# graphdeco-inria/hierarchical-3d-gaussians

Measured on NVIDIA H100. Metric: train-step images/sec (fwd+bwd) @1080p, 3M Gaussians, SH-3, higher is better.
Workload: dtype f32

## Files before the change

hierarchical-3d-gaussians_b200/csrc/common.cuh:

```cuda
#pragma once
#include <cuda_runtime.h>
#include <stdint.h>
#include <stdio.h>
#include <stdlib.h>
#include "../../include/h3dgs.h"

namespace h3dgs {

constexpr float kNearPlane = 0.2f;
constexpr float kFovClamp = 1.3f;
constexpr float kDilation = 0.3f;
constexpr float kLambdaFloor = 0.1f;
constexpr int kTile = H3DGS_TILE;
constexpr int kTilePixels = kTile * kTile;
constexpr float kAlphaCap = 0.99f;
constexpr float kAlphaSkip = 1.0f / 255.0f;
constexpr float kTStop = 0.0001f;
constexpr float kWEps = 0.0000001f;
constexpr uint32_t kKidsMask = 0xFFFFFu;
constexpr int kClampShift = 20;
constexpr uint32_t kSortedKidsMask = 0xFFFu;
constexpr int kBlockShift = 16;

struct __align__(16) Record { float4 a, b, c; };
static_assert(sizeof(Record) == 48, "record must be 48 bytes");

__host__ __device__ inline size_t align_up(size_t x, size_t a = 256) { return (x + a - 1) / a * a; }

struct GeomLayout {
    size_t depths, tiles_touched, offsets, rank_mask, records, scan_temp, total;
    size_t scan_temp_bytes;
};
struct BinLayout {
    size_t keys_unsorted, keys_sorted, vals_unsorted, vals_sorted, sort_temp, sorted_records, total;
    size_t sort_temp_bytes;
};
struct ImgLayout {
    size_t final_T, n_contrib, ranges, tile_max_contrib, tile_count, scan_info, total;
};
struct ScanInfo { uint32_t D, max_count, overflow, prefilter_bad; };
constexpr int kTileSortCap = 8192;

GeomLayout geom_layout(int P);
BinLayout bin_layout(int64_t D);
ImgLayout img_layout(int W, int H);

void prof_begin(int stage, cudaStream_t s);
void prof_end(int stage, cudaStream_t s);
struct ProfScope {
    int stage; cudaStream_t s;
    ProfScope(int st, cudaStream_t ss) : stage(st), s(ss) { prof_begin(stage, s); }
    ~ProfScope() { prof_end(stage, s); }
};

int pinned_scratch(void** out);

void set_error(const char* fmt, ...);
extern int64_t g_launches;

#define H3_CUDA(call)                                                                      \
    do {                                                                                   \
        cudaError_t e__ = (call);                                                          \
        if (e__ != cudaSuccess) {                                                          \
            h3dgs::set_error("%s failed at %s:%d: %s", #call, __FILE__, __LINE__,          \
                             cudaGetErrorString(e__));                                     \
            return H3DGS_ECUDA;                                                            \
        }                                                                                  \
    } while (0)

#define H3_LAUNCHED(name, debug, stream)                                                   \
    do {                                                                                   \
        h3dgs::g_launches++;                                                               \
        cudaError_t e__ = cudaGetLastError();                                              \
        if (e__ == cudaSuccess && (debug)) e__ = cudaStreamSynchronize(stream);            \
        if (e__ != cudaSuccess) {                                                          \
            h3dgs::set_error("kernel %s failed: %s", name, cudaGetErrorString(e__));       \
            return H3DGS_ECUDA;                                                            \
        }                                                                                  \
    } while (0)

int launch_preprocess(const h3dgs_raster_args& a, int32_t* radii, float* depths, uint32_t* tiles_touched,
                      uint8_t* rank_mask, Record* records, uint32_t* tile_count, ScanInfo* info, cudaStream_t s);
int launch_tile_scan(const h3dgs_raster_args& a, const uint32_t* tile_count, uint32_t* ranges, ScanInfo* info,
                     uint32_t cap_entries, uint32_t cap_list, cudaStream_t s);
int launch_tile_binning(const h3dgs_raster_args& a, const int32_t* radii, const float* depths, const Record* records,
                        int64_t D, uint32_t max_count, uint8_t* bin, const BinLayout& bl, const uint32_t* ranges,
                        const ScanInfo* info, uint32_t* tile_count, cudaStream_t s);
int launch_preprocess_color(const h3dgs_raster_args& a, const int32_t* radii, const uint32_t* tiles_touched,
                            Record* records, cudaStream_t s);
int launch_sh_backward(const h3dgs_raster_args& a, const int32_t* radii, const uint8_t* rank_mask, const Record* records,
                       const float* accum, float* dL_dmeans3D, float* dL_dsh, cudaStream_t s);
int launch_scan(const uint32_t* in, uint32_t* out, int n, void* temp, size_t temp_bytes, cudaStream_t s, bool debug);
size_t scan_temp_bytes(int n);
size_t sort_temp_bytes(int64_t n);
int launch_binning(const h3dgs_raster_args& a, const int32_t* radii, const float* depths, const uint32_t* offsets,
                   const Record* records, int64_t D, uint8_t* bin, const BinLayout& bl, uint32_t* ranges,
                   cudaStream_t s);
int launch_render_forward(const h3dgs_raster_args& a, const uint32_t* ranges, const Record* sorted_records,
                          float* out_color, float* out_invdepth, float* final_T, uint32_t* n_contrib,
                          uint32_t* tile_max_contrib, cudaStream_t s);
int launch_render_backward(const h3dgs_raster_args& a, const uint32_t* ranges, const Record* sorted_records,
                           const uint32_t* point_list, const float* final_T, const uint32_t* n_contrib,
                           const uint32_t* tile_max_contrib, const float* dL_dcolor, const float* dL_dinvdepth,
                           float* accum , cudaStream_t s);
int launch_preprocess_backward(const h3dgs_raster_args& a, const int32_t* radii, const uint8_t* rank_mask, const Record* records,
                               const float* accum, float* dL_dmeans3D, float* dL_dmeans2D, float* dL_dsh,
                               float* dL_dcolors, float* dL_dopacities, float* dL_dscales, float* dL_drots,
                               float* dL_dcov3D, cudaStream_t s);

#ifdef __CUDACC__
__device__ __forceinline__ void quad_pixel(int tile_x, int tile_y, int warp, int lane, int& px, int& py0) {
    px = tile_x * kTile + 8 * (warp & 1) + (lane & 7);
    py0 = tile_y * kTile + 8 * (warp >> 1) + 2 * (lane >> 3);
}

__device__ __forceinline__ void group_pixel(int tile_x, int tile_y, int warp, int lane, int& px, int& py0) {
    const int g = lane >> 3, k = lane & 7;
    px = tile_x * kTile + 8 * (warp & 1) + 4 * (g & 1) + (k & 3);
    py0 = tile_y * kTile + 8 * (warp >> 1) + 4 * (g >> 1) + 2 * (k >> 2);
}
inline bool use_group_walk() { const char* e = getenv("H3DGS_GROUPWALK"); return !(e && e[0] == '0'); }

#endif

struct PeerPtrs { void* p[H3DGS_MAX_PEERS]; int n; };
inline PeerPtrs peer_ptrs(void* const* src, int n) {
    PeerPtrs r; r.n = n > 1 ? n : 0;
    for (int k = 0; k < H3DGS_MAX_PEERS; k++) r.p[k] = (k < r.n) ? src[k] : nullptr;
    return r;
}
struct RowCycle { int shift, world, rank; };
inline RowCycle row_cycle(const h3dgs_raster_args& a) {
    RowCycle c; c.world = a.peer_count > 1 ? a.peer_count : 0; c.rank = a.shard_index; c.shift = a.grad_cyclic_log2;
    return c;
}
inline int cyclic_local_rows(const RowCycle& c, int P) {
    const int blocks = (P + (1 << c.shift) - 1) >> c.shift;
    return ((blocks + c.world - 1 - c.rank) / c.world) << c.shift;
}
#ifdef __CUDACC__
__device__ __forceinline__ int cyclic_row(const RowCycle& c, int local) {
    return ((((local >> c.shift) * c.world + c.rank)) << c.shift) + (local & ((1 << c.shift) - 1));
}
__device__ __forceinline__ bool cyclic_owned(const RowCycle& c, int row) { return ((row >> c.shift) % c.world) == c.rank; }
#endif

#ifdef __CUDACC__
struct StagePtrs { const float* own; const float* stage; int n, rank; size_t slot_floats; };
template <int NPAIR>
__device__ __forceinline__ void gather_accum_pairs(const StagePtrs& sp, uint32_t mask, int i, int first, float (&out)[2 * NPAIR]) {
#pragma unroll
    for (int k = 0; k < 2 * NPAIR; k++) out[k] = 0.f;
#pragma unroll
    for (int r = 0; r < H3DGS_MAX_PEERS; r++) {
        if (r < sp.n && ((mask >> r) & 1u)) {
            const float* row = (r == sp.rank ? sp.own : sp.stage + (size_t)r * sp.slot_floats) + (size_t)i * 10 + 2 * first;
#pragma unroll
            for (int k = 0; k < NPAIR; k++) {
                const float2 v = __ldcg(reinterpret_cast<const float2*>(row + 2 * k));
                out[2 * k] += v.x; out[2 * k + 1] += v.y;
            }
        }
    }
}
#endif
inline StagePtrs stage_ptrs(const h3dgs_raster_args& a, const float* accum) {
    StagePtrs sp; sp.own = accum; sp.n = a.peer_count > 1 ? a.peer_count : 0; sp.rank = a.shard_index;
    sp.stage = sp.n ? static_cast<const float*>(a.peer_stage[a.shard_index]) : nullptr;
    sp.slot_floats = (size_t)a.P * 10;
    return sp;
}
int launch_peer_push(const h3dgs_raster_args& a, const uint8_t* rank_mask, const float* accum, cudaStream_t s);

#ifdef H3_SIMT_EMU
extern long long g_emu_stats[16];
#define H3_STAT(i, n) (h3dgs::g_emu_stats[i] += (n))
#else
#define H3_STAT(i, n) ((void)0)
#endif

constexpr int kAccum = 10;

}

#ifdef __CUDACC__
#include "pair_math.cuh"
#endif
```

hierarchical-3d-gaussians_b200/csrc/pair_math.cuh:

```cuda
#pragma once

#ifdef H3_PAIR_HOST_EMU
#include <math.h>
#include <stdint.h>
#define H3_PM_FN static inline
namespace h3dgs {
#ifndef H3_SIMT_EMU
struct float4 { float x, y, z, w; };
constexpr float kAlphaCap = 0.99f;
constexpr float kAlphaSkip = 1.0f / 255.0f;
constexpr float kTStop = 0.0001f;
constexpr uint32_t kSortedKidsMask = 0xFFFu;
#endif
struct f2 { float lo, hi; };
H3_PM_FN f2 pk(float lo, float hi) { return f2{lo, hi}; }
H3_PM_FN void upk(f2 v, float& lo, float& hi) { lo = v.lo; hi = v.hi; }
H3_PM_FN f2 fma2(f2 a, f2 b, f2 c) { return f2{fmaf(a.lo, b.lo, c.lo), fmaf(a.hi, b.hi, c.hi)}; }
H3_PM_FN f2 mul2(f2 a, f2 b) { return f2{a.lo * b.lo, a.hi * b.hi}; }
H3_PM_FN f2 add2(f2 a, f2 b) { return f2{a.lo + b.lo, a.hi + b.hi}; }
H3_PM_FN f2 sub2(f2 a, f2 b) { return f2{a.lo - b.lo, a.hi - b.hi}; }
H3_PM_FN float fast_exp2(float x) { return exp2f(x); }
H3_PM_FN float fast_log2(float x) { return log2f(x); }
H3_PM_FN float rcp_approx(float x) { return 1.0f / x; }
H3_PM_FN float rsq_approx(float x) { return 1.0f / sqrtf(x); }
#else
#define H3_PM_FN __device__ __forceinline__
namespace h3dgs {
struct f2 { float lo, hi; };
H3_PM_FN f2 pk(float lo, float hi) { return f2{lo, hi}; }
H3_PM_FN void upk(f2 v, float& lo, float& hi) { lo = v.lo; hi = v.hi; }
H3_PM_FN f2 fma2(f2 a, f2 b, f2 c) { return f2{__fmaf_rn(a.lo, b.lo, c.lo), __fmaf_rn(a.hi, b.hi, c.hi)}; }
H3_PM_FN f2 mul2(f2 a, f2 b) { return f2{__fmul_rn(a.lo, b.lo), __fmul_rn(a.hi, b.hi)}; }
H3_PM_FN f2 add2(f2 a, f2 b) { return f2{__fadd_rn(a.lo, b.lo), __fadd_rn(a.hi, b.hi)}; }
H3_PM_FN f2 sub2(f2 a, f2 b) { return f2{__fsub_rn(a.lo, b.lo), __fsub_rn(a.hi, b.hi)}; }
H3_PM_FN float fast_exp2(float x) { float y; asm("ex2.approx.ftz.f32 %0, %1;" : "=f"(y) : "f"(x)); return y; }
H3_PM_FN float fast_log2(float x) { float y; asm("lg2.approx.ftz.f32 %0, %1;" : "=f"(y) : "f"(x)); return y; }
H3_PM_FN float rcp_approx(float x) { float y; asm("rcp.approx.ftz.f32 %0, %1;" : "=f"(y) : "f"(x)); return y; }
H3_PM_FN float rsq_approx(float x) { float y; asm("rsqrt.approx.ftz.f32 %0, %1;" : "=f"(y) : "f"(x)); return y; }
#endif

H3_PM_FN f2 bc(float x) { return pk(x, x); }
H3_PM_FN float lo(f2 v) { float a, b; upk(v, a, b); return a; }
H3_PM_FN float hi(f2 v) { float a, b; upk(v, a, b); return b; }
H3_PM_FN float hsum(f2 v) { float a, b; upk(v, a, b); return a + b; }
H3_PM_FN f2 sel2(bool p0, bool p1, f2 x, f2 y) {
    float x0, x1, y0, y1; upk(x, x0, x1); upk(y, y0, y1);
    return pk(p0 ? x0 : y0, p1 ? x1 : y1);
}
H3_PM_FN f2 ex2_2(f2 v) { float a, b; upk(v, a, b); return pk(fast_exp2(a), fast_exp2(b)); }
H3_PM_FN float fast_rcp(float x) { const float r = rcp_approx(x); return r * (2.0f - x * r); }
H3_PM_FN f2 rcp2(f2 x) {
    float x0, x1; upk(x, x0, x1);
    const f2 r = pk(rcp_approx(x0), rcp_approx(x1));
    return mul2(r, sub2(bc(2.0f), mul2(x, r)));
}

H3_PM_FN f2 pair_power(const float4& a, const float4& bb, float dx, f2 nfpy, f2& d) {
    d = add2(bc(a.y), nfpy);
    const float A = (a.z * dx) * (dx * -0.5f), B = -a.w * dx, C = -0.5f * bb.x;
    return fma2(fma2(bc(C), d, bc(B)), d, bc(A));
}
H3_PM_FN void pair_gauss(f2 power, float opacity, f2& G, f2& abase) {
    G = ex2_2(mul2(power, bc(1.4426950408889634f)));
    float a0, a1; upk(mul2(bc(opacity), G), a0, a1);
    abase = pk(fminf(kAlphaCap, a0), fminf(kAlphaCap, a1));
}
template <bool HIER, bool GRAD>
H3_PM_FN void pair_hier_alpha(f2 a, float t, uint32_t k , f2& alpha, f2& dadb) {
    alpha = a; dadb = bc(1.0f);
    if (!HIER) return;
    if (k <= 1u || t >= 1.0f) return;
    const float u = 1.0f - t;
    float a0, a1; upk(a, a0, a1);
    float o0, o1; upk(sub2(bc(1.0f), a), o0, o1);
    if (k == 2u) {
        const f2 r = pk(rsq_approx(o0), rsq_approx(o1));
        const f2 s = mul2(pk(o0, o1), r);
        f2 S = fma2(a, bc(0.02734375f), bc(0.0390625f));
        S = fma2(a, S, bc(0.0625f));
        S = fma2(a, S, bc(0.125f));
        S = fma2(a, S, bc(0.5f));
        const f2 omr = sel2(a0 < 0.0625f, a1 < 0.0625f, mul2(a, S), sub2(bc(1.0f), s));
        alpha = fma2(bc(u), omr, mul2(bc(t), a));
        if (GRAD) dadb = fma2(bc(0.5f * u), r, bc(t));
        return;
    }
    const float ik = fast_rcp((float)k);
    const f2 l2 = pk(fast_log2(o0), fast_log2(o1));
    f2 L = fma2(a, bc(0.2f), bc(0.25f));
    L = fma2(a, L, bc(0.33333334f));
    L = fma2(a, L, bc(0.5f));
    L = fma2(a, L, bc(1.0f));
    const f2 yn = mul2(mul2(a, L), bc(ik));
    f2 S = fma2(yn, bc(-0.041666668f), bc(0.16666667f));
    S = fma2(yn, S, bc(-0.5f));
    S = fma2(yn, S, bc(1.0f));
    const f2 omr_series = mul2(yn, S);
    const f2 omr_mufu = sub2(bc(1.0f), ex2_2(mul2(l2, bc(ik))));
    const f2 omr = sel2(a0 < 0.0625f, a1 < 0.0625f, omr_series, omr_mufu);
    alpha = fma2(bc(u), omr, mul2(bc(t), a));
    if (GRAD) dadb = fma2(bc(u * ik), ex2_2(mul2(l2, bc(ik - 1.0f))), bc(t));
}

H3_PM_FN f2 pair_blend(f2 pw, f2 al, f2& T, bool& done0, bool& done1, bool& v0, bool& v1, bool active = true) {
    const f2 tT = mul2(T, sub2(bc(1.0f), al));
    float pw0, pw1, al0, al1, tT0, tT1;
    upk(pw, pw0, pw1); upk(al, al0, al1); upk(tT, tT0, tT1);
    v0 = active && !done0 && pw0 <= 0.0f && al0 >= kAlphaSkip;
    v1 = active && !done1 && pw1 <= 0.0f && al1 >= kAlphaSkip;
    if (v0 && tT0 < kTStop) { done0 = true; v0 = false; }
    if (v1 && tT1 < kTStop) { done1 = true; v1 = false; }
    const f2 w = sel2(v0, v1, mul2(al, T), bc(0.f));
    T = sel2(v0, v1, tT, T);
    return w;
}

struct PairState { f2 T, acc; };

template <bool HIER, bool DEPTH>
H3_PM_FN void pair_grad(const float4& a, const float4& bb, float dx, f2 d, f2 G, f2 alpha, f2 dadb, f2 cg, f2 T_final,
                        f2 neg_bg_dot, f2 g0, f2 g1, f2 g2, f2 gd, PairState& st, float (&v)[10])
{
    const f2 rcp = rcp2(sub2(bc(1.0f), alpha));
    const f2 Tn = mul2(st.T, rcp);
    const f2 diff = sub2(cg, st.acc);
    const f2 dL_dalpha = fma2(mul2(T_final, rcp), neg_bg_dot, mul2(diff, Tn));
    const f2 dL_dab = HIER ? mul2(dL_dalpha, dadb) : dL_dalpha;
    const f2 w = mul2(alpha, Tn);
    st.T = Tn;
    st.acc = fma2(alpha, diff, st.acc);
    const f2 dL_dG = mul2(bc(bb.y), dL_dab);
    const f2 gdx = mul2(G, bc(dx)), gdy = mul2(G, d);
    const f2 qx = mul2(gdx, dL_dG), qy = mul2(gdy, dL_dG);
    v[0] = hsum(fma2(qy, bc(-a.w), mul2(qx, bc(-a.z))));
    v[1] = hsum(fma2(qx, bc(-a.w), mul2(qy, bc(-bb.x))));
    v[2] = hsum(qx) * dx;
    v[3] = hsum(mul2(qx, d));
    v[4] = hsum(mul2(qy, d));
    v[5] = hsum(mul2(G, dL_dab));
    v[6] = hsum(mul2(w, g0)); v[7] = hsum(mul2(w, g1)); v[8] = hsum(mul2(w, g2));
    v[9] = DEPTH ? hsum(mul2(w, gd)) : 0.f;
}

}
#undef H3_PM_FN
```

hierarchical-3d-gaussians_b200/csrc/render_backward.cu:

```cuda
#include "common.cuh"
#include "tma.cuh"

namespace h3dgs {

#ifdef H3_BLEND_OCC8
constexpr int kBwdBatch = 224;
constexpr int kBwdMinBlocks = 8;
#else
constexpr int kBwdBatch = 256;
constexpr int kBwdMinBlocks = 1;
#endif
constexpr int kBwdStages = 2;

__device__ __forceinline__ int reduce_slot(int lane) {
    if (lane & 1) return -1;
    const int b4 = (lane >> 4) & 1, b3 = (lane >> 3) & 1, b2 = (lane >> 2) & 1, b1 = (lane >> 1) & 1;
    int ai;
    if (!b3) { if (b2 && b1) return -1; ai = b2 ? 2 : b1; }
    else     { if (b2) return -1; ai = 3 + b1; }
    return 5 * b4 + ai;
}
__device__ __forceinline__ float xchg_add(float keep, float send, int mask) {
    return keep + __shfl_xor_sync(0xffffffffu, send, mask);
}
__device__ __forceinline__ f2 xchg_add2(float keep0, float send0, float keep1, float send1, int mask) {
    return add2(pk(keep0, keep1), pk(__shfl_xor_sync(0xffffffffu, send0, mask), __shfl_xor_sync(0xffffffffu, send1, mask)));
}
__device__ __forceinline__ float transpose_reduce10(const float (&v)[10], int lane) {
    const bool b4 = lane & 16, b3 = lane & 8, b2 = lane & 4, b1 = lane & 2;
    float a[5];
    upk(xchg_add2(b4 ? v[5] : v[0], b4 ? v[0] : v[5], b4 ? v[6] : v[1], b4 ? v[1] : v[6], 16), a[0], a[1]);
    upk(xchg_add2(b4 ? v[7] : v[2], b4 ? v[2] : v[7], b4 ? v[8] : v[3], b4 ? v[3] : v[8], 16), a[2], a[3]);
    a[4] = xchg_add(b4 ? v[9] : v[4], b4 ? v[4] : v[9], 16);
    float b[3];
    upk(xchg_add2(b3 ? a[3] : a[0], b3 ? a[0] : a[3], b3 ? a[4] : a[1], b3 ? a[1] : a[4], 8), b[0], b[1]);
    b[2] = xchg_add(b3 ? 0.f : a[2], b3 ? a[2] : 0.f, 8);
    float c[2];
    upk(xchg_add2(b2 ? b[2] : b[0], b2 ? b[0] : b[2], b2 ? 0.f : b[1], b2 ? b[1] : 0.f, 4), c[0], c[1]);
    float d = xchg_add(b1 ? c[1] : c[0], b1 ? c[0] : c[1], 2);
    d += __shfl_xor_sync(0xffffffffu, d, 1);
    return d;
}

__device__ __forceinline__ void group_slots(int k, int& s0, int& s1) {
    const int b2 = (k >> 2) & 1, b1 = (k >> 1) & 1, b0 = k & 1, base = 5 * b2;
    if (!b0) { s0 = base + (b1 ? 3 : 0); s1 = base + (b1 ? 4 : 1); }
    else { s0 = b1 ? -1 : base + 2; s1 = -1; }
}
__device__ __forceinline__ void transpose_reduce10_g8(const float (&v)[10], int lane, float& r0, float& r1) {
    const bool b2 = lane & 4, b1 = lane & 2, b0 = lane & 1;
    float a[5];
    upk(xchg_add2(b2 ? v[5] : v[0], b2 ? v[0] : v[5], b2 ? v[6] : v[1], b2 ? v[1] : v[6], 4), a[0], a[1]);
    upk(xchg_add2(b2 ? v[7] : v[2], b2 ? v[2] : v[7], b2 ? v[8] : v[3], b2 ? v[3] : v[8], 4), a[2], a[3]);
    a[4] = xchg_add(b2 ? v[9] : v[4], b2 ? v[4] : v[9], 4);
    float b[3];
    upk(xchg_add2(b1 ? a[3] : a[0], b1 ? a[0] : a[3], b1 ? a[4] : a[1], b1 ? a[1] : a[4], 2), b[0], b[1]);
    b[2] = xchg_add(b1 ? 0.f : a[2], b1 ? a[2] : 0.f, 2);
    upk(xchg_add2(b0 ? b[2] : b[0], b0 ? b[0] : b[2], b0 ? 0.f : b[1], b0 ? b[1] : 0.f, 1), r0, r1);
}

constexpr int kBwdThreads = 128;

template <bool HIER, bool DEPTH, bool GROUPS>
__global__ void __launch_bounds__(kBwdThreads, kBwdMinBlocks)
render_backward_kernel(int W, int H, int gx, int shard_count, int shard_index, const uint2* __restrict__ ranges,
                       const Record* __restrict__ sorted, const uint32_t* __restrict__ point_list,
                       const float* __restrict__ bg, const float* __restrict__ final_T,
                       const uint32_t* __restrict__ n_contrib, const uint32_t* __restrict__ tile_max_contrib,
                       const float* __restrict__ dL_dcolor, const float* __restrict__ dL_dinvdepth,
                       float* __restrict__ accum)
{
    __shared__ __align__(128) Record s_rec[kBwdStages][kBwdBatch];
    __shared__ uint32_t s_id[kBwdStages][kBwdBatch];
    __shared__ __align__(8) uint64_t s_full[kBwdStages];
    __shared__ uint8_t s_list[GROUPS ? kBwdThreads / 32 : 1][4][GROUPS ? kBwdBatch : 4];

    const int tid = threadIdx.x, lane = tid & 31, warp = tid >> 5;
    const int slot = reduce_slot(lane);
    const int tile_x = blockIdx.x % gx;
    const int tile_y = (blockIdx.x / gx) * shard_count + shard_index;
    const int tile = tile_y * gx + tile_x;
    const uint2 range = ranges[tile];
    const int n = min((int)(range.y - range.x), (int)tile_max_contrib[tile]);
    const int nb = (n + kBwdBatch - 1) / kBwdBatch;
    if (nb == 0) return;
    const Record* src = sorted + range.x;
    const uint32_t* ids = point_list + range.x;

    auto stage_ids = [&](int it) {
        const int b = nb - 1 - it, st = it % kBwdStages;
        for (int k = tid; k < kBwdBatch; k += kBwdThreads) {
            const int e = b * kBwdBatch + k;
            if (e < n) s_id[st][k] = ids[e];
        }
    };
    for (int it = 0; it < kBwdStages && it < nb; it++) stage_ids(it);
    if (tid == 0) {
        for (int s = 0; s < kBwdStages; s++) mbar_init(&s_full[s], 1);
        fence_mbar_init();
    }
    __syncthreads();
    auto issue = [&](int it) {
        const int b = nb - 1 - it, st = it % kBwdStages;
        const uint32_t bytes = (uint32_t)min(kBwdBatch, n - b * kBwdBatch) * (uint32_t)sizeof(Record);
        mbar_arrive_expect_tx(&s_full[st], bytes);
        tma_load_1d(&s_rec[st][0], src + (size_t)b * kBwdBatch, bytes, &s_full[st]);
    };
    if (tid == 0)
        for (int it = 0; it < kBwdStages && it < nb; it++) issue(it);

    int px, py0;
    if (GROUPS) group_pixel(tile_x, tile_y, warp, lane, px, py0);
    else quad_pixel(tile_x, tile_y, warp, lane, px, py0);
    int gs0, gs1;
    group_slots(lane & 7, gs0, gs1);
    const int grp = lane >> 3;
    const int py1 = py0 + 1;
    const bool in0 = px < W && py0 < H, in1 = px < W && py1 < H;
    const float fpx = (float)px;
    const f2 nfpy = pk(-(float)py0, -(float)py1);
    const size_t pix0 = (size_t)py0 * W + px, pix1 = (size_t)py1 * W + px, plane = (size_t)H * W;
    const float Tf0 = in0 ? final_T[pix0] : 0.f, Tf1 = in1 ? final_T[pix1] : 0.f;
    const f2 Tf = pk(Tf0, Tf1);
    PairState ps = {Tf, bc(0.f)};
    const int last0 = in0 ? (int)n_contrib[pix0] : 0, last1 = in1 ? (int)n_contrib[pix1] : 0;
    float ga0 = 0.f, ga1 = 0.f, ga2 = 0.f, gad = 0.f, gb0 = 0.f, gb1 = 0.f, gb2 = 0.f, gbd = 0.f;
    if (in0) { ga0 = dL_dcolor[pix0]; ga1 = dL_dcolor[plane + pix0]; ga2 = dL_dcolor[2 * plane + pix0]; if (DEPTH) gad = dL_dinvdepth[pix0]; }
    if (in1) { gb0 = dL_dcolor[pix1]; gb1 = dL_dcolor[plane + pix1]; gb2 = dL_dcolor[2 * plane + pix1]; if (DEPTH) gbd = dL_dinvdepth[pix1]; }
    const f2 g0 = pk(ga0, gb0), g1 = pk(ga1, gb1), g2 = pk(ga2, gb2), gd = pk(gad, gbd);
    const f2 neg_bgd = pk(-(bg[0] * ga0 + bg[1] * ga1 + bg[2] * ga2), -(bg[0] * gb0 + bg[1] * gb1 + bg[2] * gb2));
    const int wlast = (int)__reduce_max_sync(0xffffffffu, (unsigned)max(last0, last1));
    const int qsel = kBlockShift + 4 * warp;
    int gl0, gl1, gl2, gl3;
    {
        int gm = max(last0, last1);
        gm = max(gm, __shfl_xor_sync(0xffffffffu, gm, 4)); gm = max(gm, __shfl_xor_sync(0xffffffffu, gm, 2));
        gm = max(gm, __shfl_xor_sync(0xffffffffu, gm, 1));
        gl0 = __shfl_sync(0xffffffffu, gm, 0); gl1 = __shfl_sync(0xffffffffu, gm, 8);
        gl2 = __shfl_sync(0xffffffffu, gm, 16); gl3 = __shfl_sync(0xffffffffu, gm, 24);
    }

    for (int it = 0; it < nb; it++) {
        const int st = it % kBwdStages, b = nb - 1 - it;
        mbar_wait(&s_full[st], (uint32_t)((it / kBwdStages) & 1));
        const int cnt = min(kBwdBatch, n - b * kBwdBatch);
        const Record* rec = &s_rec[st][0];
        auto replay_entry = [&](int j, bool has) {
            const int e = b * kBwdBatch + j;
            const float4 a = rec[j].a;
            const float4 bb = rec[j].b;
            const uint32_t gid = s_id[st][j];
            const uint32_t kb = __float_as_uint(bb.w);
            const float dx = a.x - fpx;
            f2 d, G, al, dadb = bc(1.0f);
            const f2 pw = pair_power(a, bb, dx, nfpy, d);
            pair_gauss(pw, bb.y, G, al);
            float pw0, pw1, al0, al1;
            upk(pw, pw0, pw1); upk(al, al0, al1);
            bool v0 = has && e < last0 && pw0 <= 0.0f && al0 >= kAlphaSkip;
            bool v1 = has && e < last1 && pw1 <= 0.0f && al1 >= kAlphaSkip;
            if (lane == 0) H3_STAT(0, 1);
            if ((lane & 7) == 0 && has) H3_STAT(3, 1);
            if (!__any_sync(0xffffffffu, v0 || v1)) { if (lane == 0) H3_STAT(1, 1); return; }
            if (HIER) {
                pair_hier_alpha<HIER, true>(al, bb.z, kb & kSortedKidsMask, al, dadb);
                upk(al, al0, al1);
                v0 = v0 && al0 >= kAlphaSkip;
                v1 = v1 && al1 >= kAlphaSkip;
            }
            H3_STAT(2, (v0 ? 1 : 0) + (v1 ? 1 : 0));
#ifdef H3_SIMT_EMU
            { const uint32_t tk = __ballot_sync(0xffffffffu, v0 || v1);
              if (GROUPS && (lane & 7) == 0 && has && ((tk >> (8 * grp)) & 0xFFu) == 0u) H3_STAT(4, 1); }
#endif
            G = sel2(v0, v1, G, bc(0.f));
            al = sel2(v0, v1, al, bc(0.f));
            const float4 c = rec[j].c;
            f2 cg = fma2(bc(c.z), g2, fma2(bc(c.y), g1, mul2(bc(c.x), g0)));
            if (DEPTH) cg = fma2(bc(c.w), gd, cg);
            float v[10];
            pair_grad<HIER, DEPTH>(a, bb, dx, d, G, al, dadb, cg, Tf, neg_bgd, g0, g1, g2, gd, ps, v);
            if (GROUPS) {
                const bool taker = ((__ballot_sync(0xffffffffu, v0 || v1) >> (8 * grp)) & 0xFFu) != 0u;
                float r0, r1;
                transpose_reduce10_g8(v, lane, r0, r1);
                float* row = accum + (size_t)gid * kAccum;
                if (taker && gs0 >= 0 && (DEPTH || gs0 < 9)) atomicAdd(row + gs0, r0);
                if (taker && gs1 >= 0 && (DEPTH || gs1 < 9)) atomicAdd(row + gs1, r1);
            } else {
                const float total = transpose_reduce10(v, lane);
                float* row = accum + (size_t)gid * kAccum;
                if (slot >= 0 && (DEPTH || slot < 9)) atomicAdd(row + slot, total);
            }
        };
        if (GROUPS) {
            uint8_t* lst = &s_list[warp][0][0];
            const uint32_t lt = (1u << lane) - 1u;
            int c0 = 0, c1 = 0, c2 = 0, c3 = 0;
            for (int j0 = 0; j0 < cnt; j0 += 32) {
                const int jl = j0 + lane, e = b * kBwdBatch + jl;
                uint32_t nib = jl < cnt ? (__float_as_uint(rec[jl].b.w) >> qsel) & 0xFu : 0u;
                nib &= (e < gl0 ? 1u : 0u) | (e < gl1 ? 2u : 0u) | (e < gl2 ? 4u : 0u) | (e < gl3 ? 8u : 0u);
                const uint32_t m0 = __ballot_sync(0xffffffffu, nib & 1u), m1 = __ballot_sync(0xffffffffu, nib & 2u);
                const uint32_t m2 = __ballot_sync(0xffffffffu, nib & 4u), m3 = __ballot_sync(0xffffffffu, nib & 8u);
                if (nib & 1u) lst[c0 + __popc(m0 & lt)] = (uint8_t)jl;
                if (nib & 2u) lst[kBwdBatch + c1 + __popc(m1 & lt)] = (uint8_t)jl;
                if (nib & 4u) lst[2 * kBwdBatch + c2 + __popc(m2 & lt)] = (uint8_t)jl;
                if (nib & 8u) lst[3 * kBwdBatch + c3 + __popc(m3 & lt)] = (uint8_t)jl;
                c0 += __popc(m0); c1 += __popc(m1); c2 += __popc(m2); c3 += __popc(m3);
            }
            __syncwarp();
            const int mylen = grp == 0 ? c0 : grp == 1 ? c1 : grp == 2 ? c2 : c3;
            const int maxlen = max(max(c0, c1), max(c2, c3));
            const uint8_t* my = lst + grp * kBwdBatch;
            for (int i = maxlen - 1; i >= 0; i--) {
                const bool has = i < mylen;
                replay_entry(has ? (int)my[i] : 0, has);
            }
            __syncwarp();
        } else {
            for (int j0 = (cnt - 1) & ~31; j0 >= 0; j0 -= 32) {
                const int jl = j0 + lane;
                const uint32_t nib = (jl < cnt && (b * kBwdBatch + jl) < wlast) ? (__float_as_uint(rec[jl].b.w) >> qsel) & 0xFu : 0u;
                uint32_t m = __ballot_sync(0xffffffffu, nib != 0u);
                while (m != 0u) {
                    const int top = 31 - __clz(m);
                    m &= ~(1u << top);
                    replay_entry(j0 + top, true);
                }
            }
        }
        __syncthreads();
        if (it + kBwdStages < nb) {
            if (tid == 0) issue(it + kBwdStages);
            stage_ids(it + kBwdStages);
        }
    }
}

int launch_render_backward(const h3dgs_raster_args& a, const uint32_t* ranges, const Record* sorted_records,
                           const uint32_t* point_list, const float* final_T, const uint32_t* n_contrib,
                           const uint32_t* tile_max_contrib, const float* dL_dcolor, const float* dL_dinvdepth,
                           float* accum, cudaStream_t s)
{
    const int W = a.image_width, H = a.image_height;
    const int gx = (W + kTile - 1) / kTile, gy = (H + kTile - 1) / kTile;
    const int sc = a.shard_count > 0 ? a.shard_count : 1, si = a.shard_count > 0 ? a.shard_index : 0;
    const int rows = (gy + sc - 1 - si) / sc;
    if (rows <= 0 || gx <= 0) return H3DGS_OK;
    const bool hier = a.interpolation_weights != nullptr;
    const bool depth = a.do_depth != 0 && dL_dinvdepth != nullptr;
    const dim3 grid(gx * rows), block(kBwdThreads);
    ProfScope prof(H3DGS_STAGE_RENDER_BWD, s);
    const bool groups = use_group_walk();
#define LAUNCH(HI, DE, GR)                                                                                          \
    render_backward_kernel<HI, DE, GR><<<grid, block, 0, s>>>(W, H, gx, sc, si, (const uint2*)ranges, sorted_records, \
                                                              point_list, a.bg, final_T, n_contrib, tile_max_contrib, \
                                                              dL_dcolor, dL_dinvdepth, accum)
#define LAUNCH2(HI, DE) do { if (groups) LAUNCH(HI, DE, true); else LAUNCH(HI, DE, false); } while (0)
    if (hier) { if (depth) LAUNCH2(true, true); else LAUNCH2(true, false); }
    else      { if (depth) LAUNCH2(false, true); else LAUNCH2(false, false); }
#undef LAUNCH2
#undef LAUNCH
    H3_LAUNCHED("render_backward", a.debug, s);
    return H3DGS_OK;
}

}
```

hierarchical-3d-gaussians_b200/csrc/render_forward.cu:

```cuda
#include "common.cuh"
#include "tma.cuh"

namespace h3dgs {

#ifdef H3_BLEND_OCC8
constexpr int kFwdBatch = 224;
constexpr int kFwdMinBlocks = 8;
#else
constexpr int kFwdBatch = 256;
constexpr int kFwdMinBlocks = 1;
#endif
constexpr int kFwdStages = 2;

constexpr int kFwdThreads = 128;

template <bool HIER, bool DEPTH, bool GROUPS>
__global__ void __launch_bounds__(kFwdThreads, kFwdMinBlocks)
render_forward_kernel(int W, int H, int gx, int shard_count, int shard_index, const uint2* __restrict__ ranges,
                      const Record* __restrict__ sorted, const float* __restrict__ bg, float* __restrict__ out_color,
                      float* __restrict__ out_invdepth, float* __restrict__ final_T, uint32_t* __restrict__ n_contrib,
                      uint32_t* __restrict__ tile_max_contrib, const PeerPtrs peers)
{
    __shared__ __align__(128) Record s_rec[kFwdStages][kFwdBatch];
    __shared__ __align__(8) uint64_t s_full[kFwdStages];
    __shared__ uint32_t s_max;
    __shared__ uint8_t s_list[GROUPS ? kFwdThreads / 32 : 1][4][GROUPS ? kFwdBatch : 4];

    const int tid = threadIdx.x, warp = tid >> 5, lane = tid & 31;
    const int tile_x = blockIdx.x % gx;
    const int tile_y = (blockIdx.x / gx) * shard_count + shard_index;
    const int tile = tile_y * gx + tile_x;
    const uint2 range = ranges[tile];
    const int n = (int)(range.y - range.x);
    const int nb = (n + kFwdBatch - 1) / kFwdBatch;
    const Record* src = sorted + range.x;

    if (tid == 0) {
        for (int s = 0; s < kFwdStages; s++) mbar_init(&s_full[s], 1);
        s_max = 0;
        fence_mbar_init();
    }
    __syncthreads();
    int issued = 0;
    if (tid == 0) {
        for (int s = 0; s < kFwdStages && s < nb; s++) {
            const uint32_t bytes = (uint32_t)min(kFwdBatch, n - s * kFwdBatch) * (uint32_t)sizeof(Record);
            mbar_arrive_expect_tx(&s_full[s], bytes);
            tma_load_1d(&s_rec[s][0], src + (size_t)s * kFwdBatch, bytes, &s_full[s]);
        }
    }
    issued = min(kFwdStages, nb);

    int px, py0;
    if (GROUPS) group_pixel(tile_x, tile_y, warp, lane, px, py0);
    else quad_pixel(tile_x, tile_y, warp, lane, px, py0);
    const int py1 = py0 + 1;
    const bool in0 = px < W && py0 < H, in1 = px < W && py1 < H;
    const float fpx = (float)px;
    const f2 nfpy = pk(-(float)py0, -(float)py1);
    bool done0 = !in0, done1 = !in1;
    f2 T = bc(1.0f);
    float Ca0 = 0.f, Ca1 = 0.f, Ca2 = 0.f, Cb0 = 0.f, Cb1 = 0.f, Cb2 = 0.f, inv0 = 0.f, inv1 = 0.f;
    uint32_t last0 = 0, last1 = 0;
    const int qsel = kBlockShift + 4 * warp;
    const int grp = lane >> 3;

    int waited = 0;
    for (int b = 0; b < nb; b++) {
        const int st = b % kFwdStages;
        mbar_wait(&s_full[st], (uint32_t)((b / kFwdStages) & 1));
        waited = b + 1;
        const int cnt = min(kFwdBatch, n - b * kFwdBatch);
        const Record* rec = &s_rec[st][0];
        const uint32_t base = (uint32_t)(b * kFwdBatch);
        auto blend_entry = [&](int j, bool has) {
            const float4 a = rec[j].a;
            const float4 bb = rec[j].b;
            const float4 c = rec[j].c;
            const uint32_t kb = __float_as_uint(bb.w);
            f2 d, G, al, unused;
            const f2 pw = pair_power(a, bb, a.x - fpx, nfpy, d);
            pair_gauss(pw, bb.y, G, al);
            pair_hier_alpha<HIER, false>(al, bb.z, kb & kSortedKidsMask, al, unused);
            bool v0, v1;
            const f2 w = pair_blend(pw, al, T, done0, done1, v0, v1, has);
            upk(fma2(bc(c.x), w, pk(Ca0, Cb0)), Ca0, Cb0);
            upk(fma2(bc(c.y), w, pk(Ca1, Cb1)), Ca1, Cb1);
            upk(fma2(bc(c.z), w, pk(Ca2, Cb2)), Ca2, Cb2);
            if (DEPTH) upk(fma2(bc(c.w), w, pk(inv0, inv1)), inv0, inv1);
            if (lane == 0) H3_STAT(8, 1);
            if ((lane & 7) == 0 && has) H3_STAT(10, 1);
            H3_STAT(9, (v0 ? 1 : 0) + (v1 ? 1 : 0));
            const uint32_t idx = base + (uint32_t)j + 1u;
            last0 = v0 ? idx : last0; last1 = v1 ? idx : last1;
        };
        if (GROUPS) {
            uint8_t* lst = &s_list[warp][0][0];
            const uint32_t dm = __ballot_sync(0xffffffffu, done0 && done1);
            if (dm != 0xffffffffu) {
                const uint32_t live = ((dm & 0xFFu) != 0xFFu ? 1u : 0u) | (((dm >> 8) & 0xFFu) != 0xFFu ? 2u : 0u) |
                                      (((dm >> 16) & 0xFFu) != 0xFFu ? 4u : 0u) | ((dm >> 24) != 0xFFu ? 8u : 0u);
                const uint32_t lt = (1u << lane) - 1u;
                int c0 = 0, c1 = 0, c2 = 0, c3 = 0;
                for (int j0 = 0; j0 < cnt; j0 += 32) {
                    const int jl = j0 + lane;
                    const uint32_t nib = jl < cnt ? (__float_as_uint(rec[jl].b.w) >> qsel) & live : 0u;
                    const uint32_t m0 = __ballot_sync(0xffffffffu, nib & 1u), m1 = __ballot_sync(0xffffffffu, nib & 2u);
                    const uint32_t m2 = __ballot_sync(0xffffffffu, nib & 4u), m3 = __ballot_sync(0xffffffffu, nib & 8u);
                    if (nib & 1u) lst[c0 + __popc(m0 & lt)] = (uint8_t)jl;
                    if (nib & 2u) lst[kFwdBatch + c1 + __popc(m1 & lt)] = (uint8_t)jl;
                    if (nib & 4u) lst[2 * kFwdBatch + c2 + __popc(m2 & lt)] = (uint8_t)jl;
                    if (nib & 8u) lst[3 * kFwdBatch + c3 + __popc(m3 & lt)] = (uint8_t)jl;
                    c0 += __popc(m0); c1 += __popc(m1); c2 += __popc(m2); c3 += __popc(m3);
                }
                __syncwarp();
                const int mylen = grp == 0 ? c0 : grp == 1 ? c1 : grp == 2 ? c2 : c3;
                const int maxlen = max(max(c0, c1), max(c2, c3));
                const uint8_t* my = lst + grp * kFwdBatch;
                for (int i = 0; i < maxlen; i++) {
                    const bool has = i < mylen;
                    blend_entry(has ? (int)my[i] : 0, has);
                    if ((i & 15) == 15 && __all_sync(0xffffffffu, done0 && done1)) break;
                }
                __syncwarp();
            }
        } else {
            for (int j0 = 0; j0 < cnt; j0 += 32) {
                if (__all_sync(0xffffffffu, done0 && done1)) break;
                const int jl = j0 + lane;
                const uint32_t nib = jl < cnt ? (__float_as_uint(rec[jl].b.w) >> qsel) & 0xFu : 0u;
                uint32_t m = __ballot_sync(0xffffffffu, nib != 0u);
                while (m != 0u) {
                    const int j = j0 + __ffs(m) - 1;
                    m &= m - 1;
                    blend_entry(j, true);
                }
            }
        }
        const int ndone = __syncthreads_count(done0 && done1);
        if (ndone == kFwdThreads) break;
        if (b + kFwdStages < nb) {
            if (tid == 0) {
                const int nb2 = b + kFwdStages;
                const uint32_t bytes = (uint32_t)min(kFwdBatch, n - nb2 * kFwdBatch) * (uint32_t)sizeof(Record);
                mbar_arrive_expect_tx(&s_full[st], bytes);
                tma_load_1d(&s_rec[st][0], src + (size_t)nb2 * kFwdBatch, bytes, &s_full[st]);
            }
            issued = b + kFwdStages + 1;
        }
    }
    if (tid == 0)
        for (int b = waited; b < issued; b++) mbar_wait(&s_full[b % kFwdStages], (uint32_t)((b / kFwdStages) & 1));

    const float bg0 = bg[0], bg1 = bg[1], bg2 = bg[2];
    auto store = [&](bool inside, int py, float T, float c0, float c1, float c2, float invd, uint32_t last) {
        if (!inside) return;
        const size_t pix = (size_t)py * W + px;
        final_T[pix] = T;
        n_contrib[pix] = last;
        if (peers.n > 1) {
            const size_t plane = (size_t)H * W;
            const float v0 = c0 + T * bg0, v1 = c1 + T * bg1, v2 = c2 + T * bg2;
#pragma unroll
            for (int r = 0; r < H3DGS_MAX_PEERS; r++)
                if (r < peers.n && peers.p[r]) {
                    float* o = static_cast<float*>(peers.p[r]);
                    o[pix] = v0; o[plane + pix] = v1; o[2 * plane + pix] = v2;
                }
            if (DEPTH) out_invdepth[(((size_t)(blockIdx.x / gx)) * kTile + (size_t)(py & (kTile - 1))) * W + px] = invd;
        } else if (shard_count > 1) {
            const size_t local_row = blockIdx.x / gx;
            const size_t o = ((local_row * 3) * kTile + (size_t)(py & (kTile - 1))) * W + px;
            const size_t cs = (size_t)kTile * W;
            out_color[o] = c0 + T * bg0; out_color[o + cs] = c1 + T * bg1; out_color[o + 2 * cs] = c2 + T * bg2;
            if (DEPTH) out_invdepth[(local_row * kTile + (size_t)(py & (kTile - 1))) * W + px] = invd;
        } else {
            const size_t plane = (size_t)H * W;
            out_color[pix] = c0 + T * bg0; out_color[plane + pix] = c1 + T * bg1; out_color[2 * plane + pix] = c2 + T * bg2;
            if (DEPTH) out_invdepth[pix] = invd;
        }
    };
    store(in0, py0, lo(T), Ca0, Ca1, Ca2, inv0, last0);
    store(in1, py1, hi(T), Cb0, Cb1, Cb2, inv1, last1);
    const uint32_t wmax = __reduce_max_sync(0xffffffffu, max(last0, last1));
    if (lane == 0) atomicMax(&s_max, wmax);
    __syncthreads();
    if (tid == 0) tile_max_contrib[tile] = s_max;
}

int launch_render_forward(const h3dgs_raster_args& a, const uint32_t* ranges, const Record* sorted_records,
                          float* out_color, float* out_invdepth, float* final_T, uint32_t* n_contrib,
                          uint32_t* tile_max_contrib, cudaStream_t s)
{
    const int W = a.image_width, H = a.image_height;
    const int gx = (W + kTile - 1) / kTile, gy = (H + kTile - 1) / kTile;
    const int sc = a.shard_count > 0 ? a.shard_count : 1, si = a.shard_count > 0 ? a.shard_index : 0;
    const int rows = (gy + sc - 1 - si) / sc;
    if (rows <= 0 || gx <= 0) return H3DGS_OK;
    const bool hier = a.interpolation_weights != nullptr;
    const bool depth = a.do_depth != 0;
    const dim3 grid(gx * rows), block(kFwdThreads);
    ProfScope prof(H3DGS_STAGE_RENDER_FWD, s);
    const bool groups = use_group_walk();
    const PeerPtrs peers = peer_ptrs(a.peer_image, a.peer_count);
#define LAUNCH(HI, DE, GR)                                                                                         \
    render_forward_kernel<HI, DE, GR><<<grid, block, 0, s>>>(W, H, gx, sc, si, (const uint2*)ranges, sorted_records, \
                                                             a.bg, out_color, out_invdepth, final_T, n_contrib,      \
                                                             tile_max_contrib, peers)
#define LAUNCH2(HI, DE) do { if (groups) LAUNCH(HI, DE, true); else LAUNCH(HI, DE, false); } while (0)
    if (hier) { if (depth) LAUNCH2(true, true); else LAUNCH2(true, false); }
    else      { if (depth) LAUNCH2(false, true); else LAUNCH2(false, false); }
#undef LAUNCH2
#undef LAUNCH
    H3_LAUNCHED("render_forward", a.debug, s);
    return H3DGS_OK;
}

}
```

Measured before the change: 317.7.

## Restructure backward gradient reduction and pre-sum per-pixel gradient terms

The per-pair gradient now sums the pixel-pair terms first (G*dL, d*G*dL, d^2*G*dL) and scales by opacity and dx afterwards, which removes packed multiplies. dL_dalpha is factored to use a single reciprocal multiply. The two transpose-reduce routines are replaced by one templated span_reduce in which the depth term is reduced separately. The slot computation changes to match, and the group replay list is zeroed so the loop can drop its branch. The forward render pass now defaults to the non-group pixel walk while backward keeps the group walk, which changes the forward pass's pixel-to-thread mapping.

Measured after the change: 342.6, median of 6. +7.9%, better.

```diff
diff --git a/hierarchical-3d-gaussians_b200/csrc/common.cuh b/hierarchical-3d-gaussians_b200/csrc/common.cuh
--- a/hierarchical-3d-gaussians_b200/csrc/common.cuh
+++ b/hierarchical-3d-gaussians_b200/csrc/common.cuh
@@ -119,7 +119,10 @@
     px = tile_x * kTile + 8 * (warp & 1) + 4 * (g & 1) + (k & 3);
     py0 = tile_y * kTile + 8 * (warp >> 1) + 4 * (g >> 1) + 2 * (k >> 2);
 }
-inline bool use_group_walk() { const char* e = getenv("H3DGS_GROUPWALK"); return !(e && e[0] == '0'); }
+inline bool use_group_walk(bool dflt) {
+    const char* e = getenv("H3DGS_GROUPWALK");
+    return (e && e[0]) ? e[0] != '0' : dflt;
+}
 
 #endif
 
diff --git a/hierarchical-3d-gaussians_b200/csrc/pair_math.cuh b/hierarchical-3d-gaussians_b200/csrc/pair_math.cuh
--- a/hierarchical-3d-gaussians_b200/csrc/pair_math.cuh
+++ b/hierarchical-3d-gaussians_b200/csrc/pair_math.cuh
@@ -52,7 +52,7 @@
 H3_PM_FN f2 rcp2(f2 x) {
     float x0, x1; upk(x, x0, x1);
     const f2 r = pk(rcp_approx(x0), rcp_approx(x1));
-    return mul2(r, sub2(bc(2.0f), mul2(x, r)));
+    return mul2(r, fma2(pk(-x0, -x1), r, bc(2.0f)));
 }
 
 H3_PM_FN f2 pair_power(const float4& a, const float4& bb, float dx, f2 nfpy, f2& d) {
@@ -122,24 +122,28 @@
                         f2 neg_bg_dot, f2 g0, f2 g1, f2 g2, f2 gd, PairState& st, float (&v)[10])
 {
     const f2 rcp = rcp2(sub2(bc(1.0f), alpha));
-    const f2 Tn = mul2(st.T, rcp);
     const f2 diff = sub2(cg, st.acc);
-    const f2 dL_dalpha = fma2(mul2(T_final, rcp), neg_bg_dot, mul2(diff, Tn));
+    const f2 dL_dalpha = mul2(fma2(st.T, diff, mul2(T_final, neg_bg_dot)), rcp);
     const f2 dL_dab = HIER ? mul2(dL_dalpha, dadb) : dL_dalpha;
-    const f2 w = mul2(alpha, Tn);
-    st.T = Tn;
+    st.T = mul2(st.T, rcp);
+    const f2 w = mul2(alpha, st.T);
     st.acc = fma2(alpha, diff, st.acc);
-    const f2 dL_dG = mul2(bc(bb.y), dL_dab);
-    const f2 gdx = mul2(G, bc(dx)), gdy = mul2(G, d);
-    const f2 qx = mul2(gdx, dL_dG), qy = mul2(gdy, dL_dG);
-    v[0] = hsum(fma2(qy, bc(-a.w), mul2(qx, bc(-a.z))));
-    v[1] = hsum(fma2(qx, bc(-a.w), mul2(qy, bc(-bb.x))));
-    v[2] = hsum(qx) * dx;
-    v[3] = hsum(mul2(qx, d));
-    v[4] = hsum(mul2(qy, d));
-    v[5] = hsum(mul2(G, dL_dab));
-    v[6] = hsum(mul2(w, g0)); v[7] = hsum(mul2(w, g1)); v[8] = hsum(mul2(w, g2));
-    v[9] = DEPTH ? hsum(mul2(w, gd)) : 0.f;
+    float p0, p1, d0, d1;
+    upk(mul2(G, dL_dab), p0, p1);
+    upk(d, d0, d1);
+    const float dp0 = d0 * p0, dp1 = d1 * p1;
+    const float S0 = p0 + p1, S1 = dp0 + dp1, S2 = fmaf(d0, dp0, d1 * dp1);
+    const float oS0 = bb.y * S0, oS1 = bb.y * S1, dxoS0 = dx * oS0;
+    v[0] = fmaf(-a.w, oS1, -a.z * dxoS0);
+    v[1] = fmaf(-a.w, dxoS0, -bb.x * oS1);
+    v[2] = dx * dxoS0;
+    v[3] = dx * oS1;
+    v[4] = bb.y * S2;
+    v[5] = S0;
+    float w0, w1;
+    upk(w, w0, w1);
+    v[6] = fmaf(w0, lo(g0), w1 * hi(g0)); v[7] = fmaf(w0, lo(g1), w1 * hi(g1)); v[8] = fmaf(w0, lo(g2), w1 * hi(g2));
+    if (DEPTH) v[9] = fmaf(w0, lo(gd), w1 * hi(gd));
 }
 
 }
diff --git a/hierarchical-3d-gaussians_b200/csrc/render_backward.cu b/hierarchical-3d-gaussians_b200/csrc/render_backward.cu
--- a/hierarchical-3d-gaussians_b200/csrc/render_backward.cu
+++ b/hierarchical-3d-gaussians_b200/csrc/render_backward.cu
@@ -12,52 +12,28 @@
 #endif
 constexpr int kBwdStages = 2;
 
-__device__ __forceinline__ int reduce_slot(int lane) {
-    if (lane & 1) return -1;
-    const int b4 = (lane >> 4) & 1, b3 = (lane >> 3) & 1, b2 = (lane >> 2) & 1, b1 = (lane >> 1) & 1;
-    int ai;
-    if (!b3) { if (b2 && b1) return -1; ai = b2 ? 2 : b1; }
-    else     { if (b2) return -1; ai = 3 + b1; }
-    return 5 * b4 + ai;
-}
 __device__ __forceinline__ float xchg_add(float keep, float send, int mask) {
     return keep + __shfl_xor_sync(0xffffffffu, send, mask);
 }
-__device__ __forceinline__ f2 xchg_add2(float keep0, float send0, float keep1, float send1, int mask) {
-    return add2(pk(keep0, keep1), pk(__shfl_xor_sync(0xffffffffu, send0, mask), __shfl_xor_sync(0xffffffffu, send1, mask)));
-}
-__device__ __forceinline__ float transpose_reduce10(const float (&v)[10], int lane) {
-    const bool b4 = lane & 16, b3 = lane & 8, b2 = lane & 4, b1 = lane & 2;
-    float a[5];
-    upk(xchg_add2(b4 ? v[5] : v[0], b4 ? v[0] : v[5], b4 ? v[6] : v[1], b4 ? v[1] : v[6], 16), a[0], a[1]);
-    upk(xchg_add2(b4 ? v[7] : v[2], b4 ? v[2] : v[7], b4 ? v[8] : v[3], b4 ? v[3] : v[8], 16), a[2], a[3]);
-    a[4] = xchg_add(b4 ? v[9] : v[4], b4 ? v[4] : v[9], 16);
-    float b[3];
-    upk(xchg_add2(b3 ? a[3] : a[0], b3 ? a[0] : a[3], b3 ? a[4] : a[1], b3 ? a[1] : a[4], 8), b[0], b[1]);
-    b[2] = xchg_add(b3 ? 0.f : a[2], b3 ? a[2] : 0.f, 8);
-    float c[2];
-    upk(xchg_add2(b2 ? b[2] : b[0], b2 ? b[0] : b[2], b2 ? 0.f : b[1], b2 ? b[1] : 0.f, 4), c[0], c[1]);
-    float d = xchg_add(b1 ? c[1] : c[0], b1 ? c[0] : c[1], 2);
-    d += __shfl_xor_sync(0xffffffffu, d, 1);
-    return d;
-}
-
-__device__ __forceinline__ void group_slots(int k, int& s0, int& s1) {
-    const int b2 = (k >> 2) & 1, b1 = (k >> 1) & 1, b0 = k & 1, base = 5 * b2;
-    if (!b0) { s0 = base + (b1 ? 3 : 0); s1 = base + (b1 ? 4 : 1); }
-    else { s0 = b1 ? -1 : base + 2; s1 = -1; }
-}
-__device__ __forceinline__ void transpose_reduce10_g8(const float (&v)[10], int lane, float& r0, float& r1) {
-    const bool b2 = lane & 4, b1 = lane & 2, b0 = lane & 1;
-    float a[5];
-    upk(xchg_add2(b2 ? v[5] : v[0], b2 ? v[0] : v[5], b2 ? v[6] : v[1], b2 ? v[1] : v[6], 4), a[0], a[1]);
-    upk(xchg_add2(b2 ? v[7] : v[2], b2 ? v[2] : v[7], b2 ? v[8] : v[3], b2 ? v[3] : v[8], 4), a[2], a[3]);
-    a[4] = xchg_add(b2 ? v[9] : v[4], b2 ? v[4] : v[9], 4);
-    float b[3];
-    upk(xchg_add2(b1 ? a[3] : a[0], b1 ? a[0] : a[3], b1 ? a[4] : a[1], b1 ? a[1] : a[4], 2), b[0], b[1]);
-    b[2] = xchg_add(b1 ? 0.f : a[2], b1 ? a[2] : 0.f, 2);
-    upk(xchg_add2(b0 ? b[2] : b[0], b0 ? b[0] : b[2], b0 ? 0.f : b[1], b0 ? b[1] : 0.f, 1), r0, r1);
-}
+template <int SPAN, bool DEPTH>
+__device__ __forceinline__ float span_reduce(const float (&v)[10], int lane, float& x) {
+    constexpr int top = SPAN / 2, mid = SPAN / 4, low = SPAN / 8;
+    const bool bt = lane & top, bm = lane & mid, bl = lane & low;
+    float a[4], b[2];
+#pragma unroll
+    for (int i = 0; i < 4; i++) a[i] = xchg_add(bt ? v[5 + i] : v[i], bt ? v[i] : v[5 + i], top);
+    x = DEPTH ? xchg_add(bt ? v[9] : v[4], bt ? v[4] : v[9], top) : xchg_add(v[4], v[4], top);
+#pragma unroll
+    for (int i = 0; i < 2; i++) b[i] = xchg_add(bm ? a[2 + i] : a[i], bm ? a[i] : a[2 + i], mid);
+    x = xchg_add(x, x, mid);
+    float r = xchg_add(bl ? b[1] : b[0], bl ? b[0] : b[1], low);
+    x = xchg_add(x, x, low);
+#pragma unroll
+    for (int m = low / 2; m >= 1; m /= 2) { r = xchg_add(r, r, m); x = xchg_add(x, x, m); }
+    return r;
+}
+template <int SPAN>
+__device__ __forceinline__ int span_slot(int k) { const int q = k / (SPAN / 8); return q < 4 ? q : q + 1; }
 
 constexpr int kBwdThreads = 128;
 
@@ -73,10 +49,9 @@
     __shared__ __align__(128) Record s_rec[kBwdStages][kBwdBatch];
     __shared__ uint32_t s_id[kBwdStages][kBwdBatch];
     __shared__ __align__(8) uint64_t s_full[kBwdStages];
-    __shared__ uint8_t s_list[GROUPS ? kBwdThreads / 32 : 1][4][GROUPS ? kBwdBatch : 4];
+    __shared__ __align__(16) uint8_t s_list[GROUPS ? kBwdThreads / 32 : 1][4][GROUPS ? kBwdBatch : 4];
 
     const int tid = threadIdx.x, lane = tid & 31, warp = tid >> 5;
-    const int slot = reduce_slot(lane);
     const int tile_x = blockIdx.x % gx;
     const int tile_y = (blockIdx.x / gx) * shard_count + shard_index;
     const int tile = tile_y * gx + tile_x;
@@ -95,6 +70,8 @@
         }
     };
     for (int it = 0; it < kBwdStages && it < nb; it++) stage_ids(it);
+    if (GROUPS)
+        for (int k = lane; k < kBwdBatch; k += 32) reinterpret_cast<uint32_t*>(&s_list[warp][0][0])[k] = 0u;
     if (tid == 0) {
         for (int s = 0; s < kBwdStages; s++) mbar_init(&s_full[s], 1);
         fence_mbar_init();
@@ -112,8 +89,10 @@
     int px, py0;
     if (GROUPS) group_pixel(tile_x, tile_y, warp, lane, px, py0);
     else quad_pixel(tile_x, tile_y, warp, lane, px, py0);
-    int gs0, gs1;
-    group_slots(lane & 7, gs0, gs1);
+    const int k8 = lane & 7;
+    const int slot = GROUPS ? span_slot<8>(k8)
+                            : (lane & 3) == 0 ? span_slot<32>(lane) : lane == 1 ? 4 : (DEPTH && lane == 17) ? 9 : -1;
+    const int xslot = k8 == 0 ? 4 : (DEPTH && k8 == 4) ? 9 : -1;
     const int grp = lane >> 3;
     const int py1 = py0 + 1;
     const bool in0 = px < W && py0 < H, in1 = px < W && py1 < H;
@@ -180,17 +159,16 @@
             if (DEPTH) cg = fma2(bc(c.w), gd, cg);
             float v[10];
             pair_grad<HIER, DEPTH>(a, bb, dx, d, G, al, dadb, cg, Tf, neg_bgd, g0, g1, g2, gd, ps, v);
+            float* row = accum + (size_t)gid * kAccum;
+            float x;
             if (GROUPS) {
                 const bool taker = ((__ballot_sync(0xffffffffu, v0 || v1) >> (8 * grp)) & 0xFFu) != 0u;
-                float r0, r1;
-                transpose_reduce10_g8(v, lane, r0, r1);
-                float* row = accum + (size_t)gid * kAccum;
-                if (taker && gs0 >= 0 && (DEPTH || gs0 < 9)) atomicAdd(row + gs0, r0);
-                if (taker && gs1 >= 0 && (DEPTH || gs1 < 9)) atomicAdd(row + gs1, r1);
+                const float r = span_reduce<8, DEPTH>(v, lane, x);
+                if (taker) atomicAdd(row + slot, r);
+                if (taker && xslot >= 0) atomicAdd(row + xslot, x);
             } else {
-                const float total = transpose_reduce10(v, lane);
-                float* row = accum + (size_t)gid * kAccum;
-                if (slot >= 0 && (DEPTH || slot < 9)) atomicAdd(row + slot, total);
+                const float r = span_reduce<32, DEPTH>(v, lane, x);
+                if (slot >= 0) atomicAdd(row + slot, (lane & 3) == 0 ? r : x);
             }
         };
         if (GROUPS) {
@@ -213,10 +191,7 @@
             const int mylen = grp == 0 ? c0 : grp == 1 ? c1 : grp == 2 ? c2 : c3;
             const int maxlen = max(max(c0, c1), max(c2, c3));
             const uint8_t* my = lst + grp * kBwdBatch;
-            for (int i = maxlen - 1; i >= 0; i--) {
-                const bool has = i < mylen;
-                replay_entry(has ? (int)my[i] : 0, has);
-            }
+            for (int i = maxlen - 1; i >= 0; i--) replay_entry((int)my[i], i < mylen);
             __syncwarp();
         } else {
             for (int j0 = (cnt - 1) & ~31; j0 >= 0; j0 -= 32) {
@@ -252,7 +227,7 @@
     const bool depth = a.do_depth != 0 && dL_dinvdepth != nullptr;
     const dim3 grid(gx * rows), block(kBwdThreads);
     ProfScope prof(H3DGS_STAGE_RENDER_BWD, s);
-    const bool groups = use_group_walk();
+    const bool groups = use_group_walk(true);
 #define LAUNCH(HI, DE, GR)                                                                                          \
     render_backward_kernel<HI, DE, GR><<<grid, block, 0, s>>>(W, H, gx, sc, si, (const uint2*)ranges, sorted_records, \
                                                               point_list, a.bg, final_T, n_contrib, tile_max_contrib, \
diff --git a/hierarchical-3d-gaussians_b200/csrc/render_forward.cu b/hierarchical-3d-gaussians_b200/csrc/render_forward.cu
--- a/hierarchical-3d-gaussians_b200/csrc/render_forward.cu
+++ b/hierarchical-3d-gaussians_b200/csrc/render_forward.cu
@@ -201,7 +201,7 @@
     const bool depth = a.do_depth != 0;
     const dim3 grid(gx * rows), block(kFwdThreads);
     ProfScope prof(H3DGS_STAGE_RENDER_FWD, s);
-    const bool groups = use_group_walk();
+    const bool groups = use_group_walk(false);
     const PeerPtrs peers = peer_ptrs(a.peer_image, a.peer_count);
 #define LAUNCH(HI, DE, GR)                                                                                         \
     render_forward_kernel<HI, DE, GR><<<grid, block, 0, s>>>(W, H, gx, sc, si, (const uint2*)ranges, sorted_records, \
```
